# a1q123456/image_stitching

Measured on AMD Instinct MI355X. Metric: 4K frames stitched/sec, higher is better.
Workload: dtype u8

## Files before the change

image_stitching_amd/csrc/homography.hip:

```cpp
#include "homography.h"
#include "dev_math.h"
#include <algorithm>
#include <mutex>
#include <vector>

namespace {

#ifndef MIS_PHASE0
#define MIS_PHASE0 128
#endif
constexpr int PHASE0 = MIS_PHASE0;
constexpr int RNG_TABLE = 1 << 17;
#ifndef MIS_HQ_HYPS
#define MIS_HQ_HYPS 64
#endif
constexpr int HQ_HYPS = MIS_HQ_HYPS;
constexpr int TB = 256;

struct RansacState {
    int mode;
    int n_sub;
    int iter, niters, max_good, done, best_k;
    int tail_pending;
    int draw_k, draw_fail;
    long long draw_pos;
    int spec_k, spec_fail;
    long long spec_pos;
};
__device__ __forceinline__ void ransac_reset(RansacState* st, const int mode, const int max_iters) {
    st->mode = mode;
    st->n_sub = 0; st->iter = 0; st->niters = max_iters > 1 ? max_iters : 1; st->max_good = 0; st->done = 0; st->best_k = -1; st->tail_pending = 0;
    st->draw_k = 0; st->draw_fail = 0; st->draw_pos = 0;
    st->spec_k = 0; st->spec_fail = 0; st->spec_pos = 0;
}

enum DrawPhase { DRAW_FIRST, DRAW_SECOND, DRAW_SPEC };
// ... 797 lines not shown
            }
#pragma unroll
            for (int u = 0; u < HC_UNROLL; u++)
#pragma unroll
                for (int j = 0; j < HC_HYPS; j++)
                    if (use[j]) cnt[j] += __popcll(__ballot(in[u] && is_inlier(Hf[j], M[u].x, M[u].y, m[u].x, m[u].y, thr)));
        }
#pragma unroll
        for (int j = 0; j < HC_HYPS; j++) if (k0 + j < limit) good[e0 + j] = cnt[j];
    }
}

#ifndef MIS_PS_PTS
#define MIS_PS_PTS 32
#endif
constexpr int PS_PTS = MIS_PS_PTS;
constexpr int PS_TERMS = 42;
constexpr int PS_PITCH = 43;
constexpr int PS_STAGE = PS_PTS * PS_PITCH;
constexpr size_t TAIL_DYN_LDS = sizeof(double) * 2 * PS_STAGE;
struct TailShared {
    double A[81], V[81], W[9];
    double best[9], nrm[8];
    double lm[8 + 8 + 64 + 64 + 8 + 8 + 8 + 8];
    float Hf[9];
    int indR[9], indC[9];
    int np, go;
    int bad;
    double chunk[TB * 10];
    int staged;
    int done_now;
    int base, wcnt[TB / 64];
    PROF_ONLY(int prof_rot, prof_lm;)
};
__device__ __forceinline__ float4 tail_load_point(const float* s1, const float* d1, int i) {
    const float2 dd = reinterpret_cast<const float2*>(d1)[i], ss = reinterpret_cast<const float2*>(s1)[i];
    return make_float4(dd.x, dd.y, ss.x, ss.y);
}
__device__ __forceinline__ void lds_barrier() { mis_lds_barrier(); }

__device__ __forceinline__ void wave_sync() {
    __builtin_amdgcn_fence(__ATOMIC_ACQ_REL, "wavefront");
    __builtin_amdgcn_wave_barrier();
}
__device__ __forceinline__ double jc_readlane(double v, int lane) {
    return __hiloint2double(__builtin_amdgcn_readlane(__double2hiint(v), lane), __builtin_amdgcn_readlane(__double2loint(v), lane));
}
template <int CTRL, int ROW_MASK = 0xf>
__device__ __forceinline__ double jc_max_step(double v) {
    const int hi = __double2hiint(v), lo = __double2loint(v);
    const int ohi = ROW_MASK == 0xf ? 0 : hi, olo = ROW_MASK == 0xf ? 0 : lo;
    const double o = __hiloint2double(__builtin_amdgcn_update_dpp(ohi, hi, CTRL, ROW_MASK, 0xf, false), __builtin_amdgcn_update_dpp(olo, lo, CTRL, ROW_MASK, 0xf, false));
    double r;
    asm("v_max_f64 %0, %1, %2" : "=v"(r) : "v"(v), "v"(o));
    return r;
}
__device__ __forceinline__ double jc_row_max(double v) {
    v = jc_max_step<0xB1>(v);
    v = jc_max_step<0x4E>(v);
    v = jc_max_step<0x141>(v);
    v = jc_max_step<0x140>(v);
    return v;
}

template <int n>
__device__ __forceinline__ void jacobi_eigen_coop(TailShared& S) {
// ... 503 lines not shown
            S.chunk[t] = mx;
            __syncthreads();
            if (t < 16) {
                double m = 0;
                for (int i = 0; i < TB / 16; i++) { const double o = S.chunk[t * (TB / 16) + i]; asm("v_max_f64 %0, %1, %2" : "=v"(m) : "v"(m), "v"(o)); }
                S.chunk[TB + t] = m;
            }
            __syncthreads();
            if (t == 0) {
                double m = 0;
                for (int i = 0; i < 16; i++) { const double o = S.chunk[TB + i]; asm("v_max_f64 %0, %1, %2" : "=v"(m) : "v"(m), "v"(o)); }
                sc[2] = m;
            }
        }
        __syncthreads();
        PROF_ADD(2, pn);
        PROF_LM_PASS(np);
    };
    if (t < 8) x[t] = S.best[t];
    __syncthreads();
    lm_solver_run<8>(S, 10, normal_eq);
    if (t < 8) S.best[t] = x[t];
    __syncthreads();
}

#ifndef MIS_TAIL_WAVES
#define MIS_TAIL_WAVES 3
#endif
struct TailProblem {
    int b, n; HomoCall c; RansacState* st; HomoResult* res;
    float* s1; float* d1; double* rec;
};

__device__ __forceinline__ void finish_without_loop(TailShared& S, const TailProblem& p, const int mode, const int lo, int* fin) {
    const int t = threadIdx.x, n = p.n;
    const HomoCall& c = p.c;
    if (mode == 0) {
        for (int i = t; c.mask && c.active && i < n; i += TB) c.mask[i] = 0;
        if (t == 0) { p.res->ok = 0; p.res->iters = 0; p.res->ninl = 0; p.st->done = 1; fin[p.b] = lo == 0 ? 0 : 1; }
        return;
    }
    if (t == 0) for (int i = 0; i < 9; i++) S.best[i] = 0;
    __syncthreads();
    dlt_coop(S, c.src, c.dst, 4, t < 4 ? tail_load_point(c.src, c.dst, t) : make_float4(0.f, 0.f, 0.f, 0.f), p.rec);
    const int ok = S.go;
    for (int i = t; c.mask && i < n; i += TB) c.mask[i] = ok ? 1 : 0;
    if (t == 0) { p.res->ok = ok; p.res->iters = 0; p.res->ninl = ok ? 4 : 0; if (ok) for (int i = 0; i < 9; i++) p.res->H[i] = S.best[i]; p.st->done = 1; fin[p.b] = lo == 0 ? 0 : 1; }
}

template <int MODEL_POINTS = 4>
__device__ __forceinline__ void replay_hypotheses(TailShared& S, const TailProblem& p, const int* valid, const int* good, const int lo, const int hi, const int max_iters,
                                                  const double confidence, int* fin) {
    const int t = threadIdx.x, b = p.b, n = p.n;
    RansacState* st = p.st;
    PROF_T0(rp0);
    const int nsub = st->n_sub, kmax = min(hi, nsub), cnt = max(min(kmax - lo, st->niters - st->iter), 0);
    int* gl = reinterpret_cast<int*>(S.chunk);
    int* segmax = gl + 4096;
    const bool staged = cnt <= 4096;
    const int seg = (cnt + TB - 1) / TB > 0 ? (cnt + TB - 1) / TB : 1;
    if (staged) {
        for (int i = t; i < cnt; i += TB) gl[i] = valid[(size_t)b * max_iters + lo + i] ? good[(size_t)b * max_iters + lo + i] : -1;
        __syncthreads();
        int mx = -1;
        for (int i = t * seg; i < min((t + 1) * seg, cnt); i++) mx = max(mx, gl[i]);
        segmax[t] = mx;
        __syncthreads();
    }
    if (t == 0) {
        int iter = st->iter, niters = st->niters, max_good = st->max_good, best_k = st->best_k;
        int k = lo;
        while (k < kmax && iter < niters) {
            const int off = k - lo;
            if (staged && off % seg == 0 && segmax[off / seg] <= (max_good > MODEL_POINTS - 1 ? max_good : MODEL_POINTS - 1)) {
                const int adv = min(min(seg, kmax - k), niters - iter);
                k += adv; iter += adv;
                continue;
            }
            iter++;
            const int g = staged ? gl[off] : (valid[(size_t)b * max_iters + k] ? good[(size_t)b * max_iters + k] : -1);
            if (g >= 0 && g > (max_good > MODEL_POINTS - 1 ? max_good : MODEL_POINTS - 1)) {
                best_k = k; max_good = g;
                niters = ransac_update_num_iters<MODEL_POINTS>(confidence, (double)(n - g) / n, niters);
            }
            k++;
        }
        st->iter = iter; st->niters = niters; st->max_good = max_good; st->best_k = best_k;
        if (iter >= niters || (k >= nsub && st->draw_fail) || hi >= max_iters) { S.done_now = 1; st->done = 1; fin[b] = lo == 0 ? 0 : 1; }
        PROF_REPLAY(lo, rp0);
    }
}

__device__ __forceinline__ int aff_is_inlier(const float* F, float x, float y, float X, float Y, float t) {
    const float a = ((F[0] * x + F[1] * y) + F[2]) - X;
    const float b = ((F[3] * x + F[4] * y) + F[5]) - Y;
    const float e = a * a + b * b;
    return e <= t;
}
template <bool AFFINE = false>
__device__ __forceinline__ void mask_and_compact(TailShared& S, const TailProblem& p, const float thr) {
    const int t = threadIdx.x, n = p.n;
    const HomoCall& c = p.c;
    for (int i0 = 0; i0 < n; i0 += TB) {
        int i = i0 + t, f = 0;
        if (i < n) f = AFFINE ? aff_is_inlier(S.Hf, c.src[2 * i], c.src[2 * i + 1], c.dst[2 * i], c.dst[2 * i + 1], thr)
                              : is_inlier(S.Hf, c.src[2 * i], c.src[2 * i + 1], c.dst[2 * i], c.dst[2 * i + 1], thr);
        if (c.mask && i < n) c.mask[i] = (uint8_t)f;
        unsigned long long bal = __ballot(f);
        int within = __popcll(bal & ((1ull << (t & 63)) - 1ull));
        if ((t & 63) == 0) S.wcnt[t >> 6] = __popcll(bal);
        __syncthreads();
        int off = S.base;
        for (int k = 0; k < (t >> 6); k++) off += S.wcnt[k];
        if (f) {
            p.s1[2 * (off + within)] = c.src[2 * i]; p.s1[2 * (off + within) + 1] = c.src[2 * i + 1];
            p.d1[2 * (off + within)] = c.dst[2 * i]; p.d1[2 * (off + within) + 1] = c.dst[2 * i + 1];
        }
        __syncthreads();
        if (t == 0) { int s = 0; for (int k = 0; k < TB / 64; k++) s += S.wcnt[k]; S.base += s; }
        __syncthreads();
    }
}

__device__ __forceinline__ void refine_on_inliers(TailShared& S, const TailProblem& p, const int np, const TailKind kind, const int want) {
    const int t = threadIdx.x;
    PROF_TAIL_BEGIN(S, pt);
    if (np > 0) {
        const float4 pt0 = t < np ? tail_load_point(p.s1, p.d1, t) : make_float4(0.f, 0.f, 0.f, 0.f);
        dlt_coop(S, p.s1, p.d1, np, pt0, p.rec);
        PROF_ADD(4, pt);
        lm_refine_coop(S, p.s1, p.d1, np, pt0, p.rec);
    }
    PROF_TAIL_END(S, np, kind, want, pt);
}

template <class Model>
__device__ __forceinline__ void tail_problem(TailShared& S, const Model& m, const HomoCall* calls, RansacState* states, const int* valid, const int* good, float* scr_all,
                                             HomoResult* results, int lo, int hi, int max_iters, double confidence, float thr, int* fin, TailKind kind, int want, unsigned* work_ctr) {
    if (work_ctr && blockIdx.x == 0 && threadIdx.x < WL_CTRS) work_ctr[threadIdx.x] = 0;
#if MIS_CHAIN_PRIO
    __builtin_amdgcn_s_setprio(MIS_CHAIN_PRIO);
#endif
    if (threadIdx.x == 0) { S.staged = m.staged; S.bad = 0; }
    m.reset_stages();
    __syncthreads();
    const int b = blockIdx.x, t = threadIdx.x;
    TailProblem p;
    p.b = b; p.c = calls[b]; p.n = p.c.n; p.st = states + b; p.res = results + b;
    p.s1 = scr_all + 4 * p.c.pt_off; p.d1 = p.s1 + 2 * (size_t)(p.n > 0 ? p.n : 0); p.rec = m.rec(p.c);
    RansacState* const st = p.st;
    const bool refines = kind == TAIL_REFINE_ONLY;
    if (kind == TAIL_MASK_ONLY || refines) {
        if (st->tail_pending != (refines ? 2 : 1) || fin[b] != want) return;
        __syncthreads();
    } else {
        if (st->done) return;
        const int mode = st->mode;
        if (t == 0) S.done_now = 0;
        __syncthreads();
        if (mode != 2) { m.no_loop(S, p, mode, lo, fin); return; }
        replay_hypotheses<Model::MODEL_POINTS>(S, p, valid, good, lo, hi, max_iters, confidence, fin);
        __syncthreads();
        if (!S.done_now) return;
        if (kind == TAIL_REPLAY_ONLY) { if (t == 0) st->tail_pending = 1; return; }
    }
    const int result = st->max_good > 0;
    if (!refines && t == 0) { p.res->iters = st->iter; p.res->ok = result; p.res->ninl = 0; }
    if (!result) {
        for (int i = t; p.c.mask && i < p.n; i += TB) p.c.mask[i] = 0;
        if (t == 0) st->tail_pending = 0;
        return;
    }
    if (t == 0) { m.load_best(S, p, max_iters); S.base = refines ? p.res->ninl : 0; }
    __syncthreads();
    if (!refines) mask_and_compact<Model::AFFINE>(S, p, thr);
    const int np = S.base;
    if (kind == TAIL_MASK_ONLY) {
        if (t == 0) { p.res->ninl = np; m.store(p.res, S.best); st->tail_pending = 2; }
        return;
    }
    m.refine(S, p, np, kind, want);
    if (t == 0) { m.store(p.res, S.best); p.res->ninl = np; if (refines) st->tail_pending = 0; }
}

struct HomographyTail {
    static constexpr int MODEL_POINTS = 4;
    static constexpr bool AFFINE = false;
    const double* Hc; double* rec_all; int staged;
    PROF_ONLY(unsigned long long wg_in;)
    __device__ __forceinline__ void reset_stages() const {
        if (staged)
            for (int i = threadIdx.x; i < 2 * PS_PTS; i += TB) tail_dyn[i * PS_PITCH + PS_TERMS] = 0.;
    }
    __device__ __forceinline__ double* rec(const HomoCall& c) const { return rec_all + 10 * c.pt_off; }
    __device__ __forceinline__ void no_loop(TailShared& S, const TailProblem& p, const int mode, const int lo, int* fin) const { finish_without_loop(S, p, mode, lo, fin); }
    __device__ __forceinline__ void load_best(TailShared& S, const TailProblem& p, const int max_iters) const {
        const double* hb = Hc + ((size_t)p.b * max_iters + p.st->best_k) * 9;
        for (int i = 0; i < 9; i++) { S.best[i] = hb[i]; S.Hf[i] = (float)hb[i]; }
    }
    __device__ __forceinline__ void refine(TailShared& S, const TailProblem& p, const int np, const TailKind kind, const int want) const {
        refine_on_inliers(S, p, np, kind, want);
        PROF_LAST_EXIT(kind, want, wg_in);
    }
    __device__ __forceinline__ void store(HomoResult* res, const double* best) const { for (int i = 0; i < 9; i++) res->H[i] = best[i]; }
};
__global__ __launch_bounds__(TB) __attribute__((amdgpu_waves_per_eu(MIS_TAIL_WAVES, 8))) void scan_tail_kernel(const HomoCall* calls, RansacState* states, const double* Hc, const int* valid, const int* good,
                                                       float* scr_all, double* rec_all, HomoResult* results, int lo, int hi, int max_iters,
                                                       double confidence, float thr, int* fin, TailKind kind, int want, int staged, unsigned* work_ctr) {
    PROF_FIRST_ENTRY(kind, want, wg_in);
    __shared__ TailShared S;
    tail_problem(S, HomographyTail{Hc, rec_all, staged PROF_ONLY(, wg_in)}, calls, states, valid, good, scr_all, results, lo, hi, max_iters, confidence, thr, fin, kind, want, work_ctr);
}


__device__ __forceinline__ void aff_hypothesis(const float2 p1, const float2 P1, const float2 p2, const float2 P2, double* M) {
    const double x1 = p1.x, y1 = p1.y, X1 = P1.x, Y1 = P1.y, x2 = p2.x, y2 = p2.y, X2 = P2.x, Y2 = P2.y;
    const double d = 1. / ((x1 - x2) * (x1 - x2) + (y1 - y2) * (y1 - y2));
    const double S0 = d * ((X1 - X2) * (x1 - x2) + (Y1 - Y2) * (y1 - y2));
    const double S1 = d * ((Y1 - Y2) * (x1 - x2) - (X1 - X2) * (y1 - y2));
    const double S2 = d * ((Y1 - Y2) * (x1 * y2 - x2 * y1) - (X1 * y2 - X2 * y1) * (y1 - y2) - (X1 * x2 - X2 * x1) * (x1 - x2));
    const double S3 = d * (-(X1 - X2) * (x1 * y2 - x2 * y1) - (Y1 * x2 - Y2 * x1) * (x1 - x2) - (Y1 * y2 - Y2 * y1) * (y1 - y2));
    M[0] = S0; M[1] = -S1; M[2] = S2; M[3] = S1; M[4] = S0; M[5] = S3;
}
__device__ __forceinline__ void aff_hypothesis_of(const HomoCall& c, const int* id, double* M) {
    const float2* src = reinterpret_cast<const float2*>(c.src);
    const float2* dst = reinterpret_cast<const float2*>(c.dst);
    aff_hypothesis(src[id[0]], dst[id[0]], src[id[1]], dst[id[1]], M);
}

constexpr int AD_CHUNK = 4096;
constexpr int AD_PER = AD_CHUNK / TB;
constexpr unsigned AD_IDENTITY = 2u;
__device__ __forceinline__ unsigned ad_to(unsigned e, unsigned s) { return (e >> s) & 1u; }
__device__ __forceinline__ unsigned ad_cnt(unsigned e, unsigned s) { return (e >> (s ? 17 : 2)) & 0x7fffu; }
__device__ __forceinline__ unsigned ad_then(unsigned a, unsigned b) {
    const unsigned a0 = ad_to(a, 0), a1 = ad_to(a, 1);
    return ad_to(b, a0) | (ad_to(b, a1) << 1) | ((ad_cnt(a, 0) + ad_cnt(b, a0)) << 2) | ((ad_cnt(a, 1) + ad_cnt(b, a1)) << 17);
}
__global__ __launch_bounds__(TB) void aff_draw_kernel(const HomoCall* calls, RansacState* states, int* sub_idx, const unsigned* U, unsigned long long state_T,
                                                      int max_iters, DrawPhase phase, int k_hi_arg, int2* work, unsigned* work_ctr) {
#if MIS_CHAIN_PRIO
    __builtin_amdgcn_s_setprio(MIS_CHAIN_PRIO);
#endif
    __shared__ unsigned m[AD_CHUNK + 1];
// ... 165 lines not shown
        if (with_J && t < 8) sums[t] = acc;
        else if (t == 7) sc[1] = acc;
        if (with_J) {
            S.chunk[t] = mx;
            __syncthreads();
            if (t == 0) {
                double mm = 0;
                for (int i = 0; i < TB; i++) mm = fmax(mm, S.chunk[i]);
                const double sx = sums[0], sy = sums[1], sxy = sums[2], N = (double)np;
                const double JtJ[16] = {sxy, 0, sx, sy, 0, sxy, -sy, sx, sx, -sy, N, 0, sy, sx, 0, N};
                for (int i = 0; i < 16; i++) A[i] = JtJ[i];
                for (int i = 0; i < 4; i++) v[i] = sums[3 + i];
                sc[0] = sums[7]; sc[2] = mm;
            }
        }
        __syncthreads();
    };
    if (t == 0) { x[0] = S.best[0]; x[1] = S.best[3]; x[2] = S.best[2]; x[3] = S.best[5]; }
    __syncthreads();
    lm_solver_run<4>(S, lm_iters, normal_eq);
    if (t == 0) { S.best[0] = x[0]; S.best[1] = -x[1]; S.best[2] = x[2]; S.best[3] = x[1]; S.best[4] = x[0]; S.best[5] = x[3]; }
    __syncthreads();
}

__device__ __forceinline__ void aff_store(HomoResult* res, const double* M) {
    for (int i = 0; i < 6; i++) res->H[i] = M[i];
    res->H[6] = 0; res->H[7] = 0; res->H[8] = 1;
}

struct AffinePartialTail {
    static constexpr int MODEL_POINTS = 2;
    static constexpr bool AFFINE = true;
    static constexpr int staged = 0;
    const int* sub_idx; int lm_iters;
    __device__ __forceinline__ void reset_stages() const {}
    __device__ __forceinline__ double* rec(const HomoCall&) const { return nullptr; }
    __device__ __forceinline__ void no_loop(TailShared&, const TailProblem& p, const int mode, const int lo, int* fin) const {
        const int t = threadIdx.x;
        for (int i = t; p.c.mask && p.c.active && i < p.n; i += TB) p.c.mask[i] = mode ? 1 : 0;
        if (t == 0) {
            p.res->ok = mode ? 1 : 0; p.res->iters = 0; p.res->ninl = mode ? 2 : 0;
            if (mode) { const int id[2] = {0, 1}; double M[6]; aff_hypothesis_of(p.c, id, M); aff_store(p.res, M); }
            p.st->done = 1; fin[p.b] = lo == 0 ? 0 : 1;
        }
    }
    __device__ __forceinline__ void load_best(TailShared& S, const TailProblem& p, const int max_iters) const {
        aff_hypothesis_of(p.c, sub_idx + ((size_t)p.b * max_iters + p.st->best_k) * 4, S.best);
        for (int i = 0; i < 6; i++) S.Hf[i] = (float)S.best[i];
    }
    __device__ __forceinline__ void refine(TailShared& S, const TailProblem& p, const int np, TailKind, int) const {
        if (lm_iters > 0 && np > 0) aff_lm_refine(S, p.s1, p.d1, np, lm_iters);
    }
    __device__ __forceinline__ void store(HomoResult* res, const double* best) const { aff_store(res, best); }
};
__global__ __launch_bounds__(TB) void aff_tail_kernel(const HomoCall* calls, RansacState* states, const int* sub_idx, const int* valid, const int* good, float* scr_all,
                                                      HomoResult* results, int lo, int hi, int max_iters, double confidence, float thr, int* fin, TailKind kind, int want,
                                                      int lm_iters, unsigned* work_ctr) {
    __shared__ TailShared S;
    tail_problem(S, AffinePartialTail{sub_idx, lm_iters}, calls, states, valid, good, scr_all, results, lo, hi, max_iters, confidence, thr, fin, kind, want, work_ctr);
}


struct RngTable {
    unsigned* U = nullptr;
    unsigned long long state_T = 0;
};
std::mutex g_rng_mutex;
RngTable g_rng[64];

int rng_table(MisContext* ctx, RngTable* out) {
    std::lock_guard<std::mutex> lock(g_rng_mutex);
    RngTable& r = g_rng[ctx->device & 63];
    if (!r.U) {
        std::vector<unsigned> h(RNG_TABLE);
        unsigned long long st = ~0ull;
        for (int i = 0; i < RNG_TABLE; i++) {
            st = (unsigned long long)(unsigned)st * 4164903690u + (unsigned)(st >> 32);
            h[i] = (unsigned)st;
        }
        MIS_HIP(ctx, hipMalloc((void**)&r.U, sizeof(unsigned) * RNG_TABLE));
        MIS_HIP(ctx, hipMemcpy(r.U, h.data(), sizeof(unsigned) * RNG_TABLE, hipMemcpyHostToDevice));
        r.state_T = st;
    }
    *out = r;
    return MIS_OK;
}

}

int homo_batch_reserve(MisContext* ctx, HomoBatch* b, int count, long long points, int max_iters) {
    count = std::max(count, 1); points = std::max(points, 1ll); max_iters = std::max(max_iters, 1);
    size_t off = 0;
// ... 93 lines not shown
    }
    int close(int rc) const { if (rc == MIS_OK) MIS_HIP(ctx, hipGetLastError()); return rc; }
    void draw(DrawPhase phase, hipStream_t s) const {
        if (affine) {
            hipLaunchKernelGGL(aff_draw_kernel, dim3(b->count), dim3(TB), 0, s, b->calls, (RansacState*)b->state, b->sub_idx, rt.U, rt.state_T, max_iters, phase,
                               phase == DRAW_FIRST ? p0 : max_iters, b->work, b->work_ctr);
            return;
        }
        hipLaunchKernelGGL(draw_kernel, dim3(b->count), dim3(DRAW_TB), 0, s, b->calls, (RansacState*)b->state, b->sub_idx, b->draw_idx, rt.U, rt.state_T, max_iters, phase,
                           phase == DRAW_FIRST ? p0 : max_iters, b->work, b->work_ctr, confidence);
    }
    void hypotheses() const {
        const int ncu = std::max(ctx->num_cu, 1);
        if (affine) {
            hipLaunchKernelGGL(aff_score_kernel, dim3(AH_WG_PER_CU * ncu), dim3(256), 0, st, b->calls, (RansacState*)b->state, (const int*)b->sub_idx, b->valid, b->good,
                               max_iters, thr, (const int2*)b->work, (const unsigned*)b->work_ctr);
            return;
        }
        hipLaunchKernelGGL(hyp_quad_kernel, dim3(HQ_WG_PER_CU * ncu), dim3(4 * HQ_HYPS), hq_lds, st, b->calls, (RansacState*)b->state, b->sub_idx, b->Hc, b->valid, max_iters,
                           (const int2*)b->work, b->work_ctr);
        hipLaunchKernelGGL(hyp_count_kernel, dim3(HC_WG_PER_CU * ncu), dim3(256), 0, st, b->calls, (RansacState*)b->state, (const double*)b->Hc, (const int*)b->valid, b->good,
                           max_iters, thr, (const int2*)b->work, b->work_ctr);
    }
    void scan_tail(TailKind kind, RansacPhase phase) const {
        static const bool plain = getenv("MIS_TAIL_PLAIN") != nullptr && atoi(getenv("MIS_TAIL_PLAIN")) != 0;
        const int staged = (kind == TAIL_REPLAY_ONLY || kind == TAIL_MASK_ONLY || plain) ? 0 : 1;
        const bool replay = kind == TAIL_REPLAY_FINISH || kind == TAIL_REPLAY_ONLY, second = phase == PHASE_SECOND;
        const int lo = replay && second ? p0 : 0, hi = replay && second ? max_iters : p0, want = !replay && second ? 1 : 0;
        if (affine) {
            hipLaunchKernelGGL(aff_tail_kernel, dim3(b->count), dim3(TB), 0, st, b->calls, (RansacState*)b->state, (const int*)b->sub_idx, (const int*)b->valid,
                               (const int*)b->good, b->scr, b->results, lo, hi, max_iters, confidence, thr, b->fin, kind, want, lm_iters, replay ? b->work_ctr : nullptr);
            return;
        }
        hipLaunchKernelGGL(scan_tail_kernel, dim3(b->count), dim3(TB), staged ? TAIL_DYN_LDS : (size_t)0, st, b->calls, (RansacState*)b->state, b->Hc, b->valid, b->good, b->scr,
                           b->rec, b->results, lo, hi, max_iters, confidence, thr, b->fin, kind, want, staged, replay ? b->work_ctr : nullptr);
    }
    int run_phase(RansacPhase ph, TailKind replay) const {
        if (ph == PHASE_FIRST) {
            MIS_HIP(ctx, hipMemsetAsync(b->fin, 0xff, sizeof(int) * (size_t)b->count, st));
            draw(DRAW_FIRST, st);
            if (hk.after_first_draw) MIS_HIP(ctx, hipEventRecord(hk.after_first_draw, st));
            if (hk.spec_stream && max_iters > p0 && !affine) {
                MIS_HIP(ctx, hipEventRecord(hk.spec_fork, st));
                MIS_HIP(ctx, hipStreamWaitEvent(hk.spec_stream, hk.spec_fork, 0));
                draw(DRAW_SPEC, hk.spec_stream);
                MIS_HIP(ctx, hipEventRecord(hk.spec_join, hk.spec_stream));
                if (hk.spec_mark) MIS_HIP(ctx, hipEventRecord(hk.spec_mark, hk.spec_stream));
            }
        } else {
            if (max_iters <= p0) return MIS_OK;
            if (hk.spec_stream && !affine) MIS_HIP(ctx, hipStreamWaitEvent(st, hk.spec_join, 0));
            draw(DRAW_SECOND, st);
            if (hk.after_second_draw) MIS_HIP(ctx, hipEventRecord(hk.after_second_draw, st));
        }
        hypotheses();
        scan_tail(replay, ph);
        return MIS_OK;
    }
};

}

int homo_solve(MisContext* ctx, HomoBatch* b, const HomoParams& prm, hipStream_t stream, const HomoHooks* hooks) {
    Engine e;
    int rc = e.open(ctx, b, prm, stream, hooks);
    if (rc == MIS_OK) rc = e.run_phase(PHASE_FIRST, TAIL_REPLAY_FINISH);
    if (rc == MIS_OK) rc = e.run_phase(PHASE_SECOND, TAIL_REPLAY_FINISH);
    return e.close(rc);
// ... 16 lines not shown
```

image_stitching_amd/csrc/match.hip:

```cpp
#include "common.h"
#include <thread>
#include <chrono>
#include <atomic>
#include "dev_math.h"
#include "homography.h"
#include <algorithm>
#include <vector>

namespace {

struct FeatDev {
    const uint8_t* desc;
    const MisKeyPoint* kps;
    int n, w, h;
};

#include "knn_plan.h"

constexpr int KNN_TILE = 256;
__global__ __launch_bounds__(256) void knn2_hamming_kernel(const FeatDev* feats, const PairDesc* pairs, int* idx2, float* dist2) {
    __shared__ uint4 tr[KNN_TILE * 2];
    const PairDesc pd = pairs[blockIdx.y >> 1];
    const bool fwd = (blockIdx.y & 1) == 0;
    const FeatDev Q = feats[fwd ? pd.i : pd.j], T = feats[fwd ? pd.j : pd.i];
// ... 504 lines not shown
    __syncthreads();
    for (int o = 128; o > 0; o >>= 1) { if (t < o) red[t] += red[t + o]; __syncthreads(); }
    const int off = red[0], cnt = nm[k];
    if (t == 0) host_nm[k] = cnt;
    const uint4* s = reinterpret_cast<const uint4*>(matches + pairs[k].m_off);
    uint4* d = reinterpret_cast<uint4*>(host_m + off);
    static_assert(sizeof(MisDMatch) == 16, "one 16-byte store per match");
    for (int i = t; i < cnt; i += 256) d[i] = s[i];
}

struct CopySegs { const uint8_t* src[8]; uint8_t* dst[8]; unsigned bytes[8]; int n; };
__global__ __launch_bounds__(256) void copy_segments_kernel(CopySegs c) {
    for (int k = 0; k < c.n; k++) {
        const uint8_t* s = c.src[k];
        uint8_t* d = c.dst[k];
        const unsigned nb = c.bytes[k];
        if ((((uintptr_t)s | (uintptr_t)d) & 3) == 0) {
            const unsigned nw = nb >> 2;
            for (unsigned i = blockIdx.x * 256 + threadIdx.x; i < nw; i += gridDim.x * 256) reinterpret_cast<unsigned*>(d)[i] = reinterpret_cast<const unsigned*>(s)[i];
            for (unsigned i = (nw << 2) + blockIdx.x * 256 + threadIdx.x; i < nb; i += gridDim.x * 256) d[i] = s[i];
        } else {
            for (unsigned i = blockIdx.x * 256 + threadIdx.x; i < nb; i += gridDim.x * 256) d[i] = s[i];
        }
    }
}

__global__ void second_calls_kernel(int np, const HomoCall* calls1, const HomoResult* res1, const float* scr1, const int* fin1, int want, int thresh2,
                                    HomoCall* calls2, PairOut* outs) {
    int k = blockIdx.x * blockDim.x + threadIdx.x;
    if (k >= np) return;
    const HomoCall c1 = calls1[k];
    HomoCall c;
    c.src = nullptr; c.dst = nullptr; c.mask = nullptr; c.pt_off = c1.pt_off; c.n = 0; c.active = 0;
    if (fin1[k] == want && c1.active && res1[k].ok) {
        outs[k].passed = 1;
        const int ninl = res1[k].ninl;
        if (ninl >= thresh2) {
            c.src = scr1 + 4 * c1.pt_off; c.dst = c.src + 2 * (size_t)c1.n; c.n = ninl; c.active = 1;
            outs[k].second = 1;
        }
    }
    calls2[k] = c;
}

void invert3(const double* H, double* I) {
    double d = H[0] * (H[4] * H[8] - H[5] * H[7]) - H[1] * (H[3] * H[8] - H[5] * H[6]) + H[2] * (H[3] * H[7] - H[4] * H[6]);
    if (d != 0.) d = 1. / d;
    I[0] = (H[4] * H[8] - H[5] * H[7]) * d; I[1] = (H[2] * H[7] - H[1] * H[8]) * d; I[2] = (H[1] * H[5] - H[2] * H[4]) * d;
    I[3] = (H[5] * H[6] - H[3] * H[8]) * d; I[4] = (H[0] * H[8] - H[2] * H[6]) * d; I[5] = (H[2] * H[3] - H[0] * H[5]) * d;
    I[6] = (H[3] * H[7] - H[4] * H[6]) * d; I[7] = (H[1] * H[6] - H[0] * H[7]) * d; I[8] = (H[0] * H[4] - H[1] * H[3]) * d;
}

struct Arena {
    void* p = nullptr;
    size_t bytes = 0;
    bool host = false;
    hipError_t reserve(size_t need) {
        if (need <= bytes) return hipSuccess;
        if (p) { hipError_t e = host ? hipHostFree(p) : hipFree(p); p = nullptr; bytes = 0; if (e != hipSuccess) return e; }
        need = need + need / 4 + 4096;
        hipError_t e = host ? hipHostMalloc(&p, need, hipHostMallocDefault) : hipMalloc(&p, need);
        if (e == hipSuccess) bytes = need;
        return e;
    }
    void release() { if (p) { if (host) hipHostFree(p); else hipFree(p); } p = nullptr; bytes = 0; }
};

// ... 290 lines not shown
        drop_lists();
        if (e != hipSuccess) return mis_set_error(ctx, MIS_E_HIP, "hipStreamSynchronize failed: %s (%s:%d)", hipGetErrorString(e), __FILE__, __LINE__);
        return mis_set_error(ctx, MIS_E_UNSUPPORTED, "L2 matching needs integer-valued descriptors in 0..255 (SIFT style)");
    }
    for (int k = 0; k < np; k++) {
        const PairDesc& pd = pl.pairs[k];
        const PairOut& po = h.out[k];
        const int nm = h.nm[k];
        MisMatchesInfo *a = &out[pd.i * n + pd.j], *b = &out[pd.j * n + pd.i];
        MisDMatch* bm = b->matches;
        if (po.ran_ransac) {
            a->inliers_mask = (uint8_t*)malloc((size_t)nm + 1);
            memcpy(a->inliers_mask, h.mask + pd.m_off, (size_t)nm);
        }
        if (model == MIS_MATCH_AFFINE_PARTIAL) {
            const HomoResult& ar = h.r1[k];
            a->has_H = po.ran_ransac ? ar.ok : 0;
            if (a->has_H) {
                memcpy(a->H, ar.H, sizeof(a->H));
                a->num_inliers = ar.ninl;
                a->confidence = a->num_inliers / (8 + 0.3 * nm);
            }
            *b = *a;
            b->src_img_idx = pd.j; b->dst_img_idx = pd.i;
            b->matches = bm;
            if (a->inliers_mask) {
                b->inliers_mask = (uint8_t*)malloc((size_t)nm + 1);
                memcpy(b->inliers_mask, a->inliers_mask, (size_t)nm);
            }
            if (a->has_H) invert3(a->H, b->H);
            continue;
        }
        const bool det_ok = !(fabs(det3(h.r1[k].H)) < DBL_EPSILON);
        const bool passed = po.passed && det_ok, second = po.second && det_ok;
        const HomoResult& hr = second ? (h.fin[k] == 0 ? h.r2[k] : h.r3[k]) : h.r1[k];
        a->has_H = po.ran_ransac ? hr.ok : 0;
        if (a->has_H) memcpy(a->H, hr.H, sizeof(a->H));
        a->num_inliers = passed ? h.r1[k].ninl : 0;
        if (passed) {
            double c = a->num_inliers / (8 + 0.3 * nm);
            a->confidence = c > 3. ? 0. : c;
        }
        *b = *a;
        b->src_img_idx = pd.j; b->dst_img_idx = pd.i;
        b->matches = bm;
        if (a->inliers_mask) {
            b->inliers_mask = (uint8_t*)malloc((size_t)nm + 1);
            memcpy(b->inliers_mask, a->inliers_mask, (size_t)nm);
        }
        if (a->has_H) invert3(a->H, b->H);
    }
    return MIS_OK;
}

void trace_report(MatchWorkspace* ws, std::chrono::steady_clock::time_point t_begin, std::chrono::steady_clock::time_point tq,
                  std::chrono::steady_clock::time_point ts) {
    const auto te = std::chrono::steady_clock::now();
    auto us = [](auto a, auto b) { return (double)std::chrono::duration_cast<std::chrono::microseconds>(b - a).count(); };
    fprintf(stderr, "match: enqueue %.0f us, device wait %.0f us, host assembly %.0f us\n", us(t_begin, tq), us(tq, ts), us(ts, te));
    const OwnedEvent* t = ws->tev;
    auto ms = [&](int i) { float e = 0; if (t[i].ev) hipEventElapsedTime(&e, t[0].ev, t[i].ev); return e; };
    if (!(t[0].ev && t[1].ev && t[3].ev && t[4].ev && t[5].ev && t[6].ev)) return;
    if (t[7].ev) fprintf(stderr, "match chains: main chain's second draw done %.2f\n", ms(7));
    if (t[8].ev) fprintf(stderr, "match chains: speculative draw done %.2f\n", ms(8));
    fprintf(stderr, "match chains, ms after the 2-NN pass was enqueued-behind (device events): first phase done %.2f | tails of its finishers done %.2f | main chain: second RANSAC phase done %.2f, done %.2f | side chain done %.2f | third chain done %.2f\n",
            ms(1), ms(6), ms(2), ms(3), ms(4), ms(5));
}
// ... 389 lines not shown
```

Measured before the change: 3515.

## Split tail kernel into LDS-light replay and mask kernels, defer four-point DLT

Templates the RANSAC tail on its kind and adds dedicated replay-only and mask-only kernels. These use small shared-memory structs and request 8 waves per EU, where the shared launch used the heavy TailShared. For problems with exactly four points, the four-point DLT moves from the replay launch to the refine launch through a new pending state. Host-side acceptance logic changes to match. The aim is higher occupancy and less LDS and register pressure in the frequent light phases, at the cost of more kernel variants and a changed control flow for the four-point case.

```diff
diff --git a/image_stitching_amd/csrc/homography.hip b/image_stitching_amd/csrc/homography.hip
--- a/image_stitching_amd/csrc/homography.hip
+++ b/image_stitching_amd/csrc/homography.hip
@@ -2,6 +2,7 @@
 #include "dev_math.h"
 #include <algorithm>
 #include <mutex>
+#include <type_traits>
 #include <vector>
 
 namespace {
@@ -865,6 +866,18 @@
     int done_now;
     int base, wcnt[TB / 64];
     PROF_ONLY(int prof_rot, prof_lm;)
+    __device__ __forceinline__ int* replay_stage() { return reinterpret_cast<int*>(chunk); }
+};
+constexpr int REPLAY_STAGE = 4096;
+struct ReplayShared {
+    int stage[REPLAY_STAGE + TB];
+    int done_now;
+    __device__ __forceinline__ int* replay_stage() { return stage; }
+};
+struct MaskShared {
+    double best[9];
+    float Hf[9];
+    int base, wcnt[TB / 64];
 };
 __device__ __forceinline__ float4 tail_load_point(const float* s1, const float* d1, int i) {
     const float2 dd = reinterpret_cast<const float2*>(d1)[i], ss = reinterpret_cast<const float2*>(s1)[i];
@@ -1434,32 +1447,38 @@
     float* s1; float* d1; double* rec;
 };
 
-__device__ __forceinline__ void finish_without_loop(TailShared& S, const TailProblem& p, const int mode, const int lo, int* fin) {
+__device__ __forceinline__ void finish_no_model(const TailProblem& p, const int lo, int* fin) {
+    const int t = threadIdx.x;
+    const HomoCall& c = p.c;
+    for (int i = t; c.mask && c.active && i < p.n; i += TB) c.mask[i] = 0;
+    if (t == 0) { p.res->ok = 0; p.res->iters = 0; p.res->ninl = 0; p.st->done = 1; fin[p.b] = lo == 0 ? 0 : 1; }
+}
+__device__ __forceinline__ void four_point_model(TailShared& S, const TailProblem& p) {
     const int t = threadIdx.x, n = p.n;
     const HomoCall& c = p.c;
-    if (mode == 0) {
-        for (int i = t; c.mask && c.active && i < n; i += TB) c.mask[i] = 0;
-        if (t == 0) { p.res->ok = 0; p.res->iters = 0; p.res->ninl = 0; p.st->done = 1; fin[p.b] = lo == 0 ? 0 : 1; }
-        return;
-    }
     if (t == 0) for (int i = 0; i < 9; i++) S.best[i] = 0;
     __syncthreads();
     dlt_coop(S, c.src, c.dst, 4, t < 4 ? tail_load_point(c.src, c.dst, t) : make_float4(0.f, 0.f, 0.f, 0.f), p.rec);
     const int ok = S.go;
     for (int i = t; c.mask && i < n; i += TB) c.mask[i] = ok ? 1 : 0;
-    if (t == 0) { p.res->ok = ok; p.res->iters = 0; p.res->ninl = ok ? 4 : 0; if (ok) for (int i = 0; i < 9; i++) p.res->H[i] = S.best[i]; p.st->done = 1; fin[p.b] = lo == 0 ? 0 : 1; }
-}
-
-template <int MODEL_POINTS = 4>
-__device__ __forceinline__ void replay_hypotheses(TailShared& S, const TailProblem& p, const int* valid, const int* good, const int lo, const int hi, const int max_iters,
+    if (t == 0) { p.res->ok = ok; p.res->iters = 0; p.res->ninl = ok ? 4 : 0; if (ok) for (int i = 0; i < 9; i++) p.res->H[i] = S.best[i]; }
+}
+__device__ __forceinline__ void finish_without_loop(TailShared& S, const TailProblem& p, const int mode, const int lo, int* fin) {
+    if (mode == 0) { finish_no_model(p, lo, fin); return; }
+    four_point_model(S, p);
+    if (threadIdx.x == 0) { p.st->done = 1; fin[p.b] = lo == 0 ? 0 : 1; }
+}
+
+template <int MODEL_POINTS = 4, class Shared>
+__device__ __forceinline__ void replay_hypotheses(Shared& S, const TailProblem& p, const int* valid, const int* good, const int lo, const int hi, const int max_iters,
                                                   const double confidence, int* fin) {
     const int t = threadIdx.x, b = p.b, n = p.n;
     RansacState* st = p.st;
     PROF_T0(rp0);
     const int nsub = st->n_sub, kmax = min(hi, nsub), cnt = max(min(kmax - lo, st->niters - st->iter), 0);
-    int* gl = reinterpret_cast<int*>(S.chunk);
-    int* segmax = gl + 4096;
-    const bool staged = cnt <= 4096;
+    int* gl = S.replay_stage();
+    int* segmax = gl + REPLAY_STAGE;
+    const bool staged = cnt <= REPLAY_STAGE;
     const int seg = (cnt + TB - 1) / TB > 0 ? (cnt + TB - 1) / TB : 1;
     if (staged) {
         for (int i = t; i < cnt; i += TB) gl[i] = valid[(size_t)b * max_iters + lo + i] ? good[(size_t)b * max_iters + lo + i] : -1;
@@ -1499,8 +1518,8 @@
     const float e = a * a + b * b;
     return e <= t;
 }
-template <bool AFFINE = false>
-__device__ __forceinline__ void mask_and_compact(TailShared& S, const TailProblem& p, const float thr) {
+template <bool AFFINE = false, class Shared>
+__device__ __forceinline__ void mask_and_compact(Shared& S, const TailProblem& p, const float thr) {
     const int t = threadIdx.x, n = p.n;
     const HomoCall& c = p.c;
     for (int i0 = 0; i0 < n; i0 += TB) {
@@ -1536,53 +1555,80 @@
     PROF_TAIL_END(S, np, kind, want, pt);
 }
 
-template <class Model>
-__device__ __forceinline__ void tail_problem(TailShared& S, const Model& m, const HomoCall* calls, RansacState* states, const int* valid, const int* good, float* scr_all,
-                                             HomoResult* results, int lo, int hi, int max_iters, double confidence, float thr, int* fin, TailKind kind, int want, unsigned* work_ctr) {
-    if (work_ctr && blockIdx.x == 0 && threadIdx.x < WL_CTRS) work_ctr[threadIdx.x] = 0;
+enum TailPending { PENDING_NONE = 0, PENDING_MASK = 1, PENDING_REFINE = 2, PENDING_NO_LOOP = 3 };
+template <TailKind KIND, class Model, class Shared>
+__device__ __forceinline__ void tail_problem(Shared& S, const Model& m, const HomoCall* calls, RansacState* states, const int* valid, const int* good, float* scr_all,
+                                             HomoResult* results, int lo, int hi, int max_iters, double confidence, float thr, int* fin, int want, unsigned* work_ctr) {
+    constexpr bool replays = KIND == TAIL_REPLAY_FINISH || KIND == TAIL_REPLAY_ONLY, refines = KIND == TAIL_REFINE_ONLY;
+    constexpr bool heavy = KIND == TAIL_REPLAY_FINISH || KIND == TAIL_REFINE_ONLY;
+    static_assert(!heavy || std::is_same<Shared, TailShared>::value, "a launch that can refine carries TailShared");
+    if (replays && work_ctr && blockIdx.x == 0 && threadIdx.x < WL_CTRS) work_ctr[threadIdx.x] = 0;
 #if MIS_CHAIN_PRIO
     __builtin_amdgcn_s_setprio(MIS_CHAIN_PRIO);
 #endif
-    if (threadIdx.x == 0) { S.staged = m.staged; S.bad = 0; }
-    m.reset_stages();
-    __syncthreads();
+    if constexpr (heavy) {
+        if (threadIdx.x == 0) { S.staged = m.staged; S.bad = 0; }
+        m.reset_stages();
+        __syncthreads();
+    }
     const int b = blockIdx.x, t = threadIdx.x;
     TailProblem p;
     p.b = b; p.c = calls[b]; p.n = p.c.n; p.st = states + b; p.res = results + b;
-    p.s1 = scr_all + 4 * p.c.pt_off; p.d1 = p.s1 + 2 * (size_t)(p.n > 0 ? p.n : 0); p.rec = m.rec(p.c);
+    p.s1 = p.d1 = nullptr; p.rec = nullptr;
+    if constexpr (KIND != TAIL_REPLAY_ONLY) { p.s1 = scr_all + 4 * p.c.pt_off; p.d1 = p.s1 + 2 * (size_t)(p.n > 0 ? p.n : 0); }
+    if constexpr (heavy) p.rec = m.rec(p.c);
     RansacState* const st = p.st;
-    const bool refines = kind == TAIL_REFINE_ONLY;
-    if (kind == TAIL_MASK_ONLY || refines) {
-        if (st->tail_pending != (refines ? 2 : 1) || fin[b] != want) return;
-        __syncthreads();
+    if constexpr (!replays) {
+        const int pending = st->tail_pending;
+        if (fin[b] != want) return;
+        bool no_loop = false;
+        if constexpr (refines && Model::LIGHT_REPLAY) no_loop = pending == PENDING_NO_LOOP;
+        if (pending != (refines ? PENDING_REFINE : PENDING_MASK) && !no_loop) return;
+        __syncthreads();
+        if constexpr (refines && Model::LIGHT_REPLAY) {
+            if (no_loop) {
+                m.no_loop_model(S, p);
+                if (t == 0) st->tail_pending = PENDING_NONE;
+                return;
+            }
+        }
     } else {
         if (st->done) return;
         const int mode = st->mode;
         if (t == 0) S.done_now = 0;
         __syncthreads();
-        if (mode != 2) { m.no_loop(S, p, mode, lo, fin); return; }
+        if (mode != 2) {
+            if constexpr (heavy) m.no_loop(S, p, mode, lo, fin);
+            else if constexpr (Model::LIGHT_REPLAY) {
+                if (mode == 0) finish_no_model(p, lo, fin);
+                else if (t == 0) { st->done = 1; fin[b] = lo == 0 ? 0 : 1; st->tail_pending = PENDING_NO_LOOP; p.res->ok = 0; p.res->iters = 0; p.res->ninl = 0; }
+            } else m.no_loop(S, p, mode, lo, fin);
+            return;
+        }
         replay_hypotheses<Model::MODEL_POINTS>(S, p, valid, good, lo, hi, max_iters, confidence, fin);
         __syncthreads();
         if (!S.done_now) return;
-        if (kind == TAIL_REPLAY_ONLY) { if (t == 0) st->tail_pending = 1; return; }
-    }
-    const int result = st->max_good > 0;
-    if (!refines && t == 0) { p.res->iters = st->iter; p.res->ok = result; p.res->ninl = 0; }
-    if (!result) {
-        for (int i = t; p.c.mask && i < p.n; i += TB) p.c.mask[i] = 0;
-        if (t == 0) st->tail_pending = 0;
-        return;
-    }
-    if (t == 0) { m.load_best(S, p, max_iters); S.base = refines ? p.res->ninl : 0; }
-    __syncthreads();
-    if (!refines) mask_and_compact<Model::AFFINE>(S, p, thr);
-    const int np = S.base;
-    if (kind == TAIL_MASK_ONLY) {
-        if (t == 0) { p.res->ninl = np; m.store(p.res, S.best); st->tail_pending = 2; }
-        return;
-    }
-    m.refine(S, p, np, kind, want);
-    if (t == 0) { m.store(p.res, S.best); p.res->ninl = np; if (refines) st->tail_pending = 0; }
+        if constexpr (KIND == TAIL_REPLAY_ONLY) { if (t == 0) st->tail_pending = PENDING_MASK; return; }
+    }
+    if constexpr (KIND != TAIL_REPLAY_ONLY) {
+        const int result = st->max_good > 0;
+        if (!refines && t == 0) { p.res->iters = st->iter; p.res->ok = result; p.res->ninl = 0; }
+        if (!result) {
+            for (int i = t; p.c.mask && i < p.n; i += TB) p.c.mask[i] = 0;
+            if (t == 0) st->tail_pending = PENDING_NONE;
+            return;
+        }
+        if (t == 0) { m.load_best(S, p, max_iters); S.base = refines ? p.res->ninl : 0; }
+        __syncthreads();
+        if constexpr (!refines) mask_and_compact<Model::AFFINE>(S, p, thr);
+        const int np = S.base;
+        if constexpr (KIND == TAIL_MASK_ONLY) {
+            if (t == 0) { p.res->ninl = np; m.store(p.res, S.best); st->tail_pending = PENDING_REFINE; }
+        } else {
+            m.refine(S, p, np, KIND, want);
+            if (t == 0) { m.store(p.res, S.best); p.res->ninl = np; if (refines) st->tail_pending = PENDING_NONE; }
+        }
+    }
 }
 
 struct HomographyTail {
@@ -1595,8 +1641,11 @@
             for (int i = threadIdx.x; i < 2 * PS_PTS; i += TB) tail_dyn[i * PS_PITCH + PS_TERMS] = 0.;
     }
     __device__ __forceinline__ double* rec(const HomoCall& c) const { return rec_all + 10 * c.pt_off; }
+    static constexpr bool LIGHT_REPLAY = true;
     __device__ __forceinline__ void no_loop(TailShared& S, const TailProblem& p, const int mode, const int lo, int* fin) const { finish_without_loop(S, p, mode, lo, fin); }
-    __device__ __forceinline__ void load_best(TailShared& S, const TailProblem& p, const int max_iters) const {
+    __device__ __forceinline__ void no_loop_model(TailShared& S, const TailProblem& p) const { four_point_model(S, p); }
+    template <class Shared>
+    __device__ __forceinline__ void load_best(Shared& S, const TailProblem& p, const int max_iters) const {
         const double* hb = Hc + ((size_t)p.b * max_iters + p.st->best_k) * 9;
         for (int i = 0; i < 9; i++) { S.best[i] = hb[i]; S.Hf[i] = (float)hb[i]; }
     }
@@ -1606,12 +1655,23 @@
     }
     __device__ __forceinline__ void store(HomoResult* res, const double* best) const { for (int i = 0; i < 9; i++) res->H[i] = best[i]; }
 };
+template <TailKind KIND>
 __global__ __launch_bounds__(TB) __attribute__((amdgpu_waves_per_eu(MIS_TAIL_WAVES, 8))) void scan_tail_kernel(const HomoCall* calls, RansacState* states, const double* Hc, const int* valid, const int* good,
                                                        float* scr_all, double* rec_all, HomoResult* results, int lo, int hi, int max_iters,
-                                                       double confidence, float thr, int* fin, TailKind kind, int want, int staged, unsigned* work_ctr) {
-    PROF_FIRST_ENTRY(kind, want, wg_in);
+                                                       double confidence, float thr, int* fin, int want, int staged, unsigned* work_ctr) {
+    PROF_FIRST_ENTRY(KIND, want, wg_in);
     __shared__ TailShared S;
-    tail_problem(S, HomographyTail{Hc, rec_all, staged PROF_ONLY(, wg_in)}, calls, states, valid, good, scr_all, results, lo, hi, max_iters, confidence, thr, fin, kind, want, work_ctr);
+    tail_problem<KIND>(S, HomographyTail{Hc, rec_all, staged PROF_ONLY(, wg_in)}, calls, states, valid, good, scr_all, results, lo, hi, max_iters, confidence, thr, fin, want, work_ctr);
+}
+__global__ __launch_bounds__(TB) __attribute__((amdgpu_waves_per_eu(8, 8))) void replay_tail_kernel(const HomoCall* calls, RansacState* states, const int* valid, const int* good,
+                                                       HomoResult* results, int lo, int hi, int max_iters, double confidence, int* fin, unsigned* work_ctr) {
+    __shared__ ReplayShared S;
+    tail_problem<TAIL_REPLAY_ONLY>(S, HomographyTail{nullptr, nullptr, 0 PROF_ONLY(, 0ull)}, calls, states, valid, good, nullptr, results, lo, hi, max_iters, confidence, 0.f, fin, 0, work_ctr);
+}
+__global__ __launch_bounds__(TB) __attribute__((amdgpu_waves_per_eu(8, 8))) void mask_tail_kernel(const HomoCall* calls, RansacState* states, const double* Hc, float* scr_all,
+                                                       HomoResult* results, int max_iters, float thr, int* fin, int want) {
+    __shared__ MaskShared S;
+    tail_problem<TAIL_MASK_ONLY>(S, HomographyTail{Hc, nullptr, 0 PROF_ONLY(, 0ull)}, calls, states, nullptr, nullptr, scr_all, results, 0, 0, max_iters, 0., thr, fin, want, nullptr);
 }
 
 
@@ -1843,6 +1903,7 @@
     static constexpr int MODEL_POINTS = 2;
     static constexpr bool AFFINE = true;
     static constexpr int staged = 0;
+    static constexpr bool LIGHT_REPLAY = false;
     const int* sub_idx; int lm_iters;
     __device__ __forceinline__ void reset_stages() const {}
     __device__ __forceinline__ double* rec(const HomoCall&) const { return nullptr; }
@@ -1855,7 +1916,8 @@
             p.st->done = 1; fin[p.b] = lo == 0 ? 0 : 1;
         }
     }
-    __device__ __forceinline__ void load_best(TailShared& S, const TailProblem& p, const int max_iters) const {
+    template <class Shared>
+    __device__ __forceinline__ void load_best(Shared& S, const TailProblem& p, const int max_iters) const {
         aff_hypothesis_of(p.c, sub_idx + ((size_t)p.b * max_iters + p.st->best_k) * 4, S.best);
         for (int i = 0; i < 6; i++) S.Hf[i] = (float)S.best[i];
     }
@@ -1868,7 +1930,13 @@
                                                       HomoResult* results, int lo, int hi, int max_iters, double confidence, float thr, int* fin, TailKind kind, int want,
                                                       int lm_iters, unsigned* work_ctr) {
     __shared__ TailShared S;
-    tail_problem(S, AffinePartialTail{sub_idx, lm_iters}, calls, states, valid, good, scr_all, results, lo, hi, max_iters, confidence, thr, fin, kind, want, work_ctr);
+    const AffinePartialTail m{sub_idx, lm_iters};
+    switch (kind) {
+    case TAIL_REPLAY_FINISH: tail_problem<TAIL_REPLAY_FINISH>(S, m, calls, states, valid, good, scr_all, results, lo, hi, max_iters, confidence, thr, fin, want, work_ctr); break;
+    case TAIL_REPLAY_ONLY: tail_problem<TAIL_REPLAY_ONLY>(S, m, calls, states, valid, good, scr_all, results, lo, hi, max_iters, confidence, thr, fin, want, work_ctr); break;
+    case TAIL_MASK_ONLY: tail_problem<TAIL_MASK_ONLY>(S, m, calls, states, valid, good, scr_all, results, lo, hi, max_iters, confidence, thr, fin, want, work_ctr); break;
+    case TAIL_REFINE_ONLY: tail_problem<TAIL_REFINE_ONLY>(S, m, calls, states, valid, good, scr_all, results, lo, hi, max_iters, confidence, thr, fin, want, work_ctr); break;
+    }
 }
 
 
@@ -2028,8 +2096,24 @@
                                (const int*)b->good, b->scr, b->results, lo, hi, max_iters, confidence, thr, b->fin, kind, want, lm_iters, replay ? b->work_ctr : nullptr);
             return;
         }
-        hipLaunchKernelGGL(scan_tail_kernel, dim3(b->count), dim3(TB), staged ? TAIL_DYN_LDS : (size_t)0, st, b->calls, (RansacState*)b->state, b->Hc, b->valid, b->good, b->scr,
-                           b->rec, b->results, lo, hi, max_iters, confidence, thr, b->fin, kind, want, staged, replay ? b->work_ctr : nullptr);
+        const dim3 grid(b->count), wg(TB);
+        RansacState* const states = (RansacState*)b->state;
+        switch (kind) {
+        case TAIL_REPLAY_ONLY:
+            hipLaunchKernelGGL(replay_tail_kernel, grid, wg, 0, st, b->calls, states, (const int*)b->valid, (const int*)b->good, b->results, lo, hi, max_iters, confidence, b->fin, b->work_ctr);
+            break;
+        case TAIL_MASK_ONLY:
+            hipLaunchKernelGGL(mask_tail_kernel, grid, wg, 0, st, b->calls, states, (const double*)b->Hc, b->scr, b->results, max_iters, thr, b->fin, want);
+            break;
+        case TAIL_REPLAY_FINISH:
+            hipLaunchKernelGGL(scan_tail_kernel<TAIL_REPLAY_FINISH>, grid, wg, staged ? TAIL_DYN_LDS : (size_t)0, st, b->calls, states, b->Hc, b->valid, b->good, b->scr, b->rec, b->results,
+                               lo, hi, max_iters, confidence, thr, b->fin, want, staged, b->work_ctr);
+            break;
+        case TAIL_REFINE_ONLY:
+            hipLaunchKernelGGL(scan_tail_kernel<TAIL_REFINE_ONLY>, grid, wg, staged ? TAIL_DYN_LDS : (size_t)0, st, b->calls, states, b->Hc, b->valid, b->good, b->scr, b->rec, b->results,
+                               lo, hi, max_iters, confidence, thr, b->fin, want, staged, nullptr);
+            break;
+        }
     }
     int run_phase(RansacPhase ph, TailKind replay) const {
         if (ph == PHASE_FIRST) {
diff --git a/image_stitching_amd/csrc/match.hip b/image_stitching_amd/csrc/match.hip
--- a/image_stitching_amd/csrc/match.hip
+++ b/image_stitching_amd/csrc/match.hip
@@ -560,7 +560,7 @@
     const HomoCall c1 = calls1[k];
     HomoCall c;
     c.src = nullptr; c.dst = nullptr; c.mask = nullptr; c.pt_off = c1.pt_off; c.n = 0; c.active = 0;
-    if (fin1[k] == want && c1.active && res1[k].ok) {
+    if (fin1[k] == want && c1.active && c1.n != 4 && res1[k].ok) {
         outs[k].passed = 1;
         const int ninl = res1[k].ninl;
         if (ninl >= thresh2) {
@@ -917,7 +917,8 @@
             continue;
         }
         const bool det_ok = !(fabs(det3(h.r1[k].H)) < DBL_EPSILON);
-        const bool passed = po.passed && det_ok, second = po.second && det_ok;
+        const bool four = po.ran_ransac && nm == 4;
+        const bool passed = (four ? h.r1[k].ok != 0 : po.passed != 0) && det_ok, second = po.second && det_ok;
         const HomoResult& hr = second ? (h.fin[k] == 0 ? h.r2[k] : h.r3[k]) : h.r1[k];
         a->has_H = po.ran_ransac ? hr.ok : 0;
         if (a->has_H) memcpy(a->H, hr.H, sizeof(a->H));
```

New measurement: 3556 (median of 6 runs). 1.01x the previous value.
